# Research-Implementation/AudioVidSum-A-Multi-Modal-Approach-to-Video-Summarization

Hardware: AMD Instinct MI355X
Metric: frames/sec end-to-end (extract+fuse+score), 224x224 + 16kHz (higher is better)
Workload: dtype f16x2; 1 GPU; configs[1]: SumMe-shape batch, 25 videos x ~1800 frames (45143 frames/GPU), visual-only resnet50 extractor (batch-stat BN, the reference's 4-frame BatchNorm micro-batches inside each video) + AVBiLSTM attention scorer + mean-threshold selection; frames_per_gpu=45143, videos_per_gpu=25, extractor=resnet50, frames_per_group=4, chunk_frames=16384, parallelism=videos sharded x1, no data-path collective, selected_frames_rank0=22823

## Files before the change

### audiovidsum-a-multi-modal-approach-to-video-summarization_amd/csrc/igemm.hip

```cpp
#include "avs_internal.h"
#include "igemm_params.h"
#include <type_traits>

__device__ __attribute__((aligned(16))) unsigned int avs_zero16[4];

#ifdef AVS_STUDY
#define AVS_DEBUG_BIT(p, bit) ((p).debug & (bit))
#else
#define AVS_DEBUG_BIT(p, bit) 0
#endif

#define AVS_GLDS16(src, dst)                                                                        \
  __builtin_amdgcn_global_load_lds((const __attribute__((address_space(1))) void*)(src),            \
                                   (__attribute__((address_space(3))) void*)(dst), 16, 0, 0)

__device__ __forceinline__ void avs_split_bf16(const float4& p0, const float4& p1, bf16x8& hi, bf16x8& lo) {
  const float v[8] = {p0.x, p0.y, p0.z, p0.w, p1.x, p1.y, p1.z, p1.w};
  unsigned h[4], l[4];
#pragma unroll
  for (int j = 0; j < 4; ++j) {
    const unsigned short h0 = avs_f32_to_bf16(v[2 * j]), h1 = avs_f32_to_bf16(v[2 * j + 1]);
    const unsigned short l0 = avs_f32_to_bf16(v[2 * j] - avs_bf16_to_f32(h0));
    const unsigned short l1 = avs_f32_to_bf16(v[2 * j + 1] - avs_bf16_to_f32(h1));
    h[j] = (unsigned)h0 | ((unsigned)h1 << 16);
    l[j] = (unsigned)l0 | ((unsigned)l1 << 16);
  }
  hi = __builtin_bit_cast(bf16x8, make_uint4(h[0], h[1], h[2], h[3]));
  lo = __builtin_bit_cast(bf16x8, make_uint4(l[0], l[1], l[2], l[3]));
}


template <int ES, int BN, bool ACC64, bool SPATIAL, int ROWB, int EPI, bool PIPE, int WR = 2, bool FASTK = false,
          int SPLIT = 0, bool TAP9 = false, bool AP8 = false, bool XIN = false>
__global__ __launch_bounds__(256, (ROWB == 64 && !ACC64 && WR == 2) ? ((BN == 64 && ES == 2) ? 4 : 3) : 2) void igemm_kernel(
    IgemmParams p) {
  static_assert(!AP8 || (SPLIT == 2 && ES == 4 && PIPE && ROWB == 64 && FASTK && !SPATIAL && !TAP9 && EPI == EPI_STATS),
                "AVS_F16P8 input: the AVS_F16X2 1x1 convolution + statistics on the pipelined tiles");
  static_assert(!TAP9 || (((SPLIT == 2 && ES == 4) || (SPLIT == 0 && ES == 2)) && PIPE && WR == 4 && ROWB == 64 && FASTK &&
                          SPATIAL && (EPI == EPI_STATS || EPI == EPI_BNLOCAL || (EPI == EPI_BRELU && SPLIT == 2))),
                "the shifted-row form: AVS_F16X2 / bf16 convolution + statistics / tile-local BatchNorm (3x3), AVS_F16X2 bias + "
                "ReLU (any stride-1 'same' filter) on the pipelined 256-row tiles");
  static_assert(!XIN || (TAP9 && SPLIT == 2 && EPI == EPI_STATS), "the input affine: AVS_F16X2 nine-tap convolution + statistics");
  static_assert(SPLIT == 0 || (ES == 4 && !ACC64), "the split arithmetic is for 4-byte operands");
  static_assert(WR == 2 || (WR == 4 && !ACC64 && (ES == 2 || SPLIT != 0)),
                "256-row tiles are built for the bf16 variants and the fp32-split arithmetic");
  static_assert(!PIPE || (ROWB == 64 && !ACC64), "the 3-buffer pipeline is built for the 64-byte-row variants");
  static_assert(!ACC64 || (ES == 4 && BN == 64), "fp64 slice accumulation: fp32 operands, narrow tile only");
  static_assert(ROWB == 64 || ROWB == 128, "row bytes");
  constexpr int CE = 16 / ES;
  constexpr int BKE = ROWB / ES;
  constexpr int CPRR = ROWB / 16;
  constexpr int RPP = 256 / CPRR;
  constexpr int SH = ROWB == 128 ? 1 : 2;
  constexpr int KS = ROWB / 32;
  constexpr int WC = 4 / WR;
  constexpr int WCOLS = BN / WC;
  constexpr int A_ROWS = 64 * WR;
  constexpr int NA = A_ROWS / RPP;
  constexpr int NB = (BN + RPP - 1) / RPP;
  constexpr int NT = WCOLS / 32;
  constexpr int BUF = (A_ROWS + NB * RPP) * CPRR;
  static_assert(BN == 64 || BN == 128 || (BN == 96 && SPLIT == 2 && WR == 4 && PIPE && ROWB == 64 && EPI == EPI_BRELU),
                "96-column tiles: the AVS_F16X2 bias + ReLU form on the pipelined 256-row tiles");
  static_assert(WCOLS % 32 == 0, "a wave's columns are whole 32-wide MFMA tiles");
  constexpr int CT_PITCH = BN * 2 + 16;
  constexpr int CT_SLOTS = ES == 2 ? (A_ROWS * CT_PITCH) / 16 : 0;
  constexpr int NBUF = PIPE ? 3 : 2;
  constexpr int TAB_SLOTS = EPI == EPI_BNLOCAL ? (BNLOCAL_MAX_GROUPS * 2 * BN * 4) / 16
                            : EPI == EPI_STATS ? (WR * 2 * 2 * BN * 4) / 16
                                               : 0;
  constexpr int H2_P = WCOLS + 8;
  constexpr int H2_SLOTS = SPLIT == 2 ? (4 * 32 * H2_P * 4) / 16 : 0;
  constexpr int T9_AROWS = 384;
  constexpr int T9_ABUF = (T9_AROWS + 4) * CPRR;
  constexpr int T9_BBUF = NB * RPP * CPRR;
  constexpr int OPERAND_SLOTS = TAP9 ? 2 * T9_ABUF + 3 * T9_BBUF : NBUF * BUF;
  constexpr int LDS_BASE = OPERAND_SLOTS > CT_SLOTS + TAB_SLOTS ? OPERAND_SLOTS : CT_SLOTS + TAB_SLOTS;
  constexpr int LDS_SLOTS = LDS_BASE > H2_SLOTS ? LDS_BASE : H2_SLOTS;

  __shared__ uint4 lds[LDS_SLOTS];

  const unsigned nwg = gridDim.x, orig = blockIdx.x;
  const unsigned q = nwg >> 3, rr = nwg & 7, xcd = orig & 7;
  const unsigned wg = (xcd < rr ? xcd * (q + 1) : rr * (q + 1) + (xcd - rr) * q) + (orig >> 3);
  const int tn = wg % p.tiles_n;
  const int tm = wg / p.tiles_n;
  const int m0 = EPI == EPI_BNLOCAL ? tm * p.tile_rows : tm * A_ROWS;
  const int n0 = tn * BN;

  const long long z = blockIdx.z;
  const char* __restrict__ x = p.x + z * p.sA * ES;
  const char* __restrict__ w = p.w + z * p.sB * ES;
  char* __restrict__ y = p.y + z * p.sC * ES;
  const float* __restrict__ bias = p.bias ? p.bias + z * p.sBias : nullptr;
  const char* zsrc = reinterpret_cast<const char*>(avs_zero16);

  const int t = threadIdx.x;
  const int wave = __builtin_amdgcn_readfirstlane(t >> 6), lane = t & 63;
  const int c = t & (CPRR - 1);
  const int rb = t / CPRR;
  const int cq = c ^ ((rb >> SH) & (CPRR - 1));

  const char* a_base[NA];
  int hi0[NA], wi0[NA];
#pragma unroll
  for (int i = 0; i < NA; ++i) {
    int m = m0 + rb + RPP * i;
    if constexpr (EPI == EPI_BNLOCAL) {
      if (rb + RPP * i >= p.tile_rows) m = p.M;
    }
    if (m < p.M && p.lin_stride >= 0) {
      hi0[i] = 0;
      wi0[i] = 0;
      a_base[i] = x + (long long)m * p.lin_stride * ES;
    } else if (m < p.M) {
      const int n = m / p.HoWo;
      const int rem = m - n * p.HoWo;
      const int ho = rem / p.Wo;
      const int wo = rem - ho * p.Wo;
      hi0[i] = ho * p.sh - p.ph;
      wi0[i] = wo * p.sw - p.pw;
      a_base[i] = x + ((long long)n * p.x_img_stride + (long long)hi0[i] * p.x_row_stride +
                       (long long)wi0[i] * p.x_px_stride) * ES;
    } else {
      hi0[i] = -(1 << 29);
      wi0[i] = 0;
      a_base[i] = nullptr;
    }
  }
  const char* b_base[NB];
#pragma unroll
  for (int i = 0; i < NB; ++i) {
    const int n = n0 + rb + RPP * i;
// ... 110 lines not shown
#pragma unroll
    for (int i = 0; i < NA; ++i) {
      bool ok = kval && a_base[i] != nullptr;
      if constexpr (SPATIAL)
        ok = ok && (unsigned)(hi0[i] + kh) < (unsigned)p.H && (unsigned)(wi0[i] + kw) < (unsigned)p.W;
      const unsigned long long am = ok ? ~0ull : 0ull;
      const char* src = reinterpret_cast<const char*>(
          (reinterpret_cast<unsigned long long>(a_base[i] + koff) & am) |
          (reinterpret_cast<unsigned long long>(zsrc) & ~am));
      AVS_GLDS16(src, abuf + 256 * i);
    }
#pragma unroll
    for (int i = 0; i < NB; ++i) {
      const unsigned long long bm = (kval && b_base[i] != nullptr) ? ~0ull : 0ull;
      constexpr int KSE = 64 / ES;
      const char* bsrc = p.w_kstep ? w + (((long long)(kc / KSE) * p.N + (n0 + rb + RPP * i)) * KSE + (kc % KSE)) * ES
                                   : b_base[i] + (long long)kc * ES;
      const char* src = reinterpret_cast<const char*>((reinterpret_cast<unsigned long long>(bsrc) & bm) |
                                                      (reinterpret_cast<unsigned long long>(zsrc) & ~bm));
      AVS_GLDS16(src, bbuf + 256 * i);
    }
    kc += BKE;
    ci += BKE;
    while (ci >= p.cin) {
      ci -= p.cin;
      if (++kw == p.KW) {
        kw = 0;
        ++kh;
      }
    }
  };

  const int wr = wave / WC, wc = wave % WC;
  const int lr = lane & 31, lh = lane >> 5;

  f32x16 acc[2][NT];
#pragma unroll
  for (int i = 0; i < 2; ++i)
#pragma unroll
    for (int j = 0; j < NT; ++j)
#pragma unroll
      for (int e = 0; e < 16; ++e) acc[i][j][e] = 0.f;

  double acc64[ACC64 ? 2 : 1][ACC64 ? NT : 1][ACC64 ? 16 : 1];
  if constexpr (ACC64) {
#pragma unroll
    for (int i = 0; i < 2; ++i)
#pragma unroll
      for (int j = 0; j < NT; ++j)
#pragma unroll
        for (int e = 0; e < 16; ++e) acc64[i][j][e] = 0.0;
  }

  const int steps = (p.K + BKE - 1) / BKE;
  if constexpr (TAP9) {
    constexpr int T9_NA = T9_AROWS / RPP;
    constexpr bool TGEN = EPI == EPI_BRELU;
    const int ntap = TGEN ? p.K / p.cin : 9;
    const int tkw = TGEN ? p.KW : 3;
    const int tph = TGEN ? p.ph : 1, tpw = TGEN ? p.pw : 1;
    const long long pxs = TGEN ? p.x_px_stride : (long long)p.cin;
    const unsigned lds_base = (unsigned)(unsigned long long)((__attribute__((address_space(3))) char*)lds);
    const int w1 = TGEN ? tph * p.W + tpw : p.W + 1;
    const long long mbase = m0 > w1 ? m0 - w1 : 0;
    const __amdgpu_buffer_rsrc_t a9 = __builtin_amdgcn_make_buffer_rsrc(const_cast<char*>(x) + mbase * pxs * ES, 0,
                                                                         (int)BUF_OOB, 0x00020000);
    const __amdgpu_buffer_rsrc_t b9 = __builtin_amdgcn_make_buffer_rsrc(
        const_cast<char*>(w) + (p.w_kstep ? (long long)n0 * 64 : (long long)n0 * p.ldb * ES), 0, (int)BUF_OOB, 0x00020000);
    unsigned aoff9[T9_NA], boff9[NB];
#pragma unroll
    for (int i = 0; i < T9_NA; ++i) {
      const long long m = (long long)m0 - w1 + rb + RPP * i;
      aoff9[i] = (m >= 0 && m < p.M) ? (unsigned)((m - mbase) * pxs * ES) + cq * 16 : BUF_OOB;
    }
#pragma unroll
    for (int i = 0; i < NB; ++i)
      boff9[i] = (n0 + rb + RPP * i >= p.N || rb + RPP * i >= BN) ? BUF_OOB
                 : p.w_kstep                                      ? (unsigned)((rb + RPP * i) * 64) + (cq & 3) * 16
                                                                  : (unsigned)((long long)(rb + RPP * i) * p.ldb * ES) + cq * 16;
    unsigned vm[2];
#pragma unroll
    for (int mt = 0; mt < 2; ++mt) {
      unsigned mk = 0;
      const int m = m0 + wr * 64 + mt * 32 + lr;
      bool live = m < p.M;
      if constexpr (EPI == EPI_BNLOCAL) live = live && wr * 64 + mt * 32 + lr < p.tile_rows;
      if (live) {
        const int pix = m % p.HoWo;
        const int yy = pix / p.W, xx = pix - yy * p.W;
        if constexpr (TGEN) {
          for (int tp = 0; tp < ntap; ++tp)
            if ((unsigned)(yy + tp / tkw - tph) < (unsigned)p.H && (unsigned)(xx + tp % tkw - tpw) < (unsigned)p.W) mk |= 1u << tp;
        } else {
#pragma unroll
          for (int tp = 0; tp < 9; ++tp)
            if ((unsigned)(yy + tp / 3 - 1) < (unsigned)p.H && (unsigned)(xx + tp % 3 - 1) < (unsigned)p.W) mk |= 1u << tp;
        }
      }
      vm[mt] = mk;
    }
    if (t < 32) lds[(t >> 4) * T9_ABUF + T9_AROWS * CPRR + (t & 15)] = make_uint4(0u, 0u, 0u, 0u);
    asm volatile("s_waitcnt lgkmcnt(0)" ::: "memory");
    unsigned fb9[NT][2];
#pragma unroll
    for (int nt = 0; nt < NT; ++nt)
#pragma unroll
// ... 5 lines not shown
    const int nblk = p.cin / BKE;
    auto stage_a = [&](int blk, int buf) {
      uint4* abuf = lds + buf * T9_ABUF + wave * 64;
#pragma unroll
      for (int i = 0; i < T9_NA; ++i)
        __builtin_amdgcn_raw_ptr_buffer_load_lds(a9, (__attribute__((address_space(3))) void*)(abuf + 256 * i), 16,
                                                 (int)aoff9[i], blk * ROWB, 0, 0);
    };
    int sb_blk = 0, sb_tap = 0, sb_slot = 0;
    auto stage_b = [&]() {
      uint4* bbuf = lds + 2 * T9_ABUF + sb_slot * T9_BBUF + wave * 64;
      const int kstep = sb_tap * nblk + sb_blk;
      const int kb = p.w_kstep ? kstep * (p.N * ROWB) : kstep * ROWB;
#pragma unroll
      for (int i = 0; i < NB; ++i)
        __builtin_amdgcn_raw_ptr_buffer_load_lds(b9, (__attribute__((address_space(3))) void*)(bbuf + 256 * i), 16,
                                                 (int)boff9[i], kb, 0, 0);
      sb_slot = sb_slot == 2 ? 0 : sb_slot + 1;
      if (++sb_tap == ntap) {
        sb_tap = 0;
        ++sb_blk;
      }
    };
    auto xin_block = [&](int b) {
      uint4* ab = lds + (b & 1) * T9_ABUF;
#pragma unroll
      for (int i = 0; i < (T9_AROWS * 2) / 256; ++i) {
        const int u = t + 256 * i;
        const int a = u >> 1, run = u & 1;
        const int m = m0 - w1 + a;
        if (m < 0 || m >= p.M) continue;
        const int g = m / p.rows_per_group;
        const long long ch = (long long)g * p.cin + b * BKE + run * 8;
        uint4& hi = ab[a * CPRR + ((2 * run) ^ ((a >> SH) & (CPRR - 1)))];
        uint4& lo = ab[a * CPRR + ((2 * run + 1) ^ ((a >> SH) & (CPRR - 1)))];
        float v[8], sc[8], sf[8];
        avs_f16x2_join8(hi, lo, v);
        *reinterpret_cast<float4*>(&sc[0]) = *reinterpret_cast<const float4*>(p.in_scale + ch);
        *reinterpret_cast<float4*>(&sc[4]) = *reinterpret_cast<const float4*>(p.in_scale + ch + 4);
        *reinterpret_cast<float4*>(&sf[0]) = *reinterpret_cast<const float4*>(p.in_shift + ch);
        *reinterpret_cast<float4*>(&sf[4]) = *reinterpret_cast<const float4*>(p.in_shift + ch + 4);
#pragma unroll
        for (int j = 0; j < 8; ++j) v[j] = v[j] * sc[j] + sf[j];
        if (p.in_relu) {
#pragma unroll
          for (int j = 0; j < 8; ++j) v[j] = fmaxf(v[j], 0.f);
        }
        uint4 h, l;
        avs_f16x2_split8(v, h, l);
        hi = h;
        lo = l;
      }
    };
    stage_a(0, 0);
    stage_b();
    if (steps > 1) stage_b();
    const int abase = wr * 64 + lr + w1;
    int blk = 0, tap = 0, tdx = 0, slot = 0, sig = -w1;
    for (int s = 0; s < steps; ++s) {
      if (s + 1 < steps) {
        if (tap == 1 && blk + 1 < nblk)
          asm volatile("s_waitcnt vmcnt(%0)" ::"n"(NB + T9_NA) : "memory");
        else
          asm volatile("s_waitcnt vmcnt(%0)" ::"n"(NB) : "memory");
      } else {
        asm volatile("s_waitcnt vmcnt(0)" ::: "memory");
      }
      __builtin_amdgcn_s_barrier();
      if constexpr (XIN) {
        if (tap == 0) {
          xin_block(blk);
          asm volatile("s_waitcnt lgkmcnt(0)" ::: "memory");
          __builtin_amdgcn_s_barrier();
        }
      }
      const unsigned abuf = lds_base + (unsigned)(blk & 1) * (T9_ABUF * 16u);
      const unsigned bbase = lds_base + (unsigned)(2 * T9_ABUF + slot * T9_BBUF) * 16u;
      uint4 fa[2][2], fb[2][NT];
      unsigned aaddr[2];
#pragma unroll
      for (int mt = 0; mt < 2; ++mt) {
        const int a = ((vm[mt] >> tap) & 1u) ? abase + mt * 32 + sig : T9_AROWS;
        aaddr[mt] = abuf + (unsigned)a * ROWB + (unsigned)((SPLIT == 2 ? 2 * lh : lh) ^ ((a >> SH) & (CPRR - 1))) * 16u;
      }
#pragma unroll
      for (int mt = 0; mt < 2; ++mt) fa[0][mt] = avs_lds_read_b128(aaddr[mt]);
#pragma unroll
      for (int nt = 0; nt < NT; ++nt) fb[0][nt] = avs_lds_read_b128(bbase + fb9[nt][0]);
#pragma unroll
      for (int mt = 0; mt < 2; ++mt) fa[1][mt] = avs_lds_read_b128(aaddr[mt] ^ (SPLIT == 2 ? 16u : 32u));
#pragma unroll
      for (int nt = 0; nt < NT; ++nt) fb[1][nt] = avs_lds_read_b128(bbase + fb9[nt][1]);
      if (tap == 0 && blk + 1 < nblk) stage_a(blk + 1, (blk + 1) & 1);
      if (s + 2 < steps) stage_b();
      asm volatile("s_waitcnt lgkmcnt(%0)" ::"n"(2 + NT) : "memory");
#pragma unroll
      for (int mt = 0; mt < 2; ++mt) avs_pin(fa[0][mt]);
#pragma unroll
      for (int nt = 0; nt < NT; ++nt) avs_pin(fb[0][nt]);
      __builtin_amdgcn_sched_barrier(0);
#pragma unroll
      for (int mt = 0; mt < 2; ++mt)
#pragma unroll
        for (int nt = 0; nt < NT; ++nt)
          if constexpr (SPLIT == 2)
            acc[mt][nt] = __builtin_amdgcn_mfma_f32_32x32x16_f16(__builtin_bit_cast(avs_f16x8, fa[0][mt]),
                                                                 __builtin_bit_cast(avs_f16x8, fb[0][nt]), acc[mt][nt], 0, 0, 0);
          else
            acc[mt][nt] = __builtin_amdgcn_mfma_f32_32x32x16_bf16(__builtin_bit_cast(bf16x8, fa[0][mt]),
                                                                  __builtin_bit_cast(bf16x8, fb[0][nt]), acc[mt][nt], 0, 0, 0);
      asm volatile("s_waitcnt lgkmcnt(0)" ::: "memory");
#pragma unroll
      for (int mt = 0; mt < 2; ++mt) avs_pin(fa[1][mt]);
#pragma unroll
      for (int nt = 0; nt < NT; ++nt) avs_pin(fb[1][nt]);
      __builtin_amdgcn_sched_barrier(0);
#pragma unroll
      for (int mt = 0; mt < 2; ++mt)
#pragma unroll
        for (int nt = 0; nt < NT; ++nt) {
          if constexpr (SPLIT == 2) {
            acc[mt][nt] = __builtin_amdgcn_mfma_f32_32x32x16_f16(__builtin_bit_cast(avs_f16x8, fa[1][mt]),
                                                                 __builtin_bit_cast(avs_f16x8, fb[0][nt]), acc[mt][nt], 0, 0, 0);
            acc[mt][nt] = __builtin_amdgcn_mfma_f32_32x32x16_f16(__builtin_bit_cast(avs_f16x8, fa[0][mt]),
// ... 285 lines not shown
      } else {
#pragma unroll
        for (int mt = 0; mt < 2; ++mt)
#pragma unroll
          for (int e = 0; e < 16; ++e) {
            const int roff = mt * 32 + (e & 3) + 8 * (e >> 2);
            s += (roff >= lo && roff < hi) ? acc[mt][nt][e] : 0.f;
          }
      }
      return s + __shfl_xor(s, 32, 64);
    };
    auto wave_sq = [&](int nt, int lo, int hi, float mean) -> float {
      float s = 0.f;
#pragma unroll
      for (int mt = 0; mt < 2; ++mt)
#pragma unroll
        for (int e = 0; e < 16; ++e) {
          const int roff = mt * 32 + (e & 3) + 8 * (e >> 2);
          const float d = acc[mt][nt][e] - mean;
          s = (roff >= lo && roff < hi) ? fmaf(d, d, s) : s;
        }
      return s + __shfl_xor(s, 32, 64);
    };
    float sc0[NT], sf0[NT], sc1[NT], sf1[NT], sc2[NT], sf2[NT];
    int bnd1 = 1 << 30, bnd2 = 1 << 30;
    int used = A_ROWS;
    if constexpr (EPI == EPI_BNLOCAL) used = (m0 + p.tile_rows <= p.M ? p.tile_rows : p.M - m0);
    constexpr int G = WCOLS / 8;
    constexpr int RSTEP = 64 / G;
    constexpr int NU = (32 + RSTEP - 1) / RSTEP;
    constexpr bool RAGGED = 64 % G != 0;
    static_assert(!RAGGED || EPI == EPI_BRELU, "ragged run maps: the bias + ReLU form only (no residual rows)");
    constexpr bool NORM = EPI == EPI_BNLOCAL || EPI == EPI_AFFINE || EPI == EPI_BRELU;
    float* const wreg = fl + wave * (32 * H2_P);
    const bool relu = NORM && (EPI == EPI_BRELU || p.act == AVS_ACT_RELU);
    if constexpr (EPI == EPI_BRELU) {
#pragma unroll
      for (int nt = 0; nt < NT; ++nt) {
        const int col = n0 + wc * WCOLS + nt * 32 + lr;
        sc0[nt] = 1.f;
        sf0[nt] = col < p.N ? bias[col] : 0.f;
        sc1[nt] = sc2[nt] = 1.f;
        sf1[nt] = sf2[nt] = 0.f;
      }
    }
    const int rl0 = lane / G, grp = lane % G;
    const int col8 = n0 + wc * WCOLS + grp * 8;
    const int row_lim = (EPI == EPI_BNLOCAL ? m0 + used : p.M);
    const bool col_ok = col8 < p.N && (!RAGGED || lane < RSTEP * G);
    const bool relu_l = relu && (p.relu_cols <= 0 || col8 < p.relu_cols);
    const int p8_hi = (col8 >> 4) * 48 + ((col8 >> 3) & 1) * 16;
    const int p8_rem = 32 - ((col8 >> 3) & 1) * 8;
    uint4 rhi[2][NORM ? NU : 1], rlo[2][NORM ? NU : 1];
    auto res_fetch = [&](auto half) {
      constexpr int mt = decltype(half)::value;
      if constexpr (NORM) {
        const long long row0 = (long long)m0 + wr * 64 + mt * 32 + rl0;
        if (EPI == EPI_AFFINE && p.res_p8) {
          const char* base = p.residual + row0 * p.ldr * 3 + p8_hi;
          const long long step = (long long)RSTEP * p.ldr * 3;
#pragma unroll
          for (int it = 0; it < NU; ++it) {
            const bool ok = col_ok && row0 + it * RSTEP < row_lim;
            const char* rp = ok ? base + it * step : p.residual + p8_hi;
            rhi[mt][it] = *reinterpret_cast<const uint4*>(rp);
            const uint2 q = *reinterpret_cast<const uint2*>(rp + p8_rem);
            rlo[mt][it] = make_uint4(q.x, q.y, 0u, 0u);
          }
          return;
        }
        const char* base = p.residual + (row0 * p.ldr + col8) * 4;
        const long long step = (long long)RSTEP * p.ldr * 4;
#pragma unroll
        for (int it = 0; it < NU; ++it) {
          const bool ok = col_ok && row0 + it * RSTEP < row_lim;
          const uint4* rp = reinterpret_cast<const uint4*>(ok ? base + it * step : p.residual);
          rhi[mt][it] = rp[0];
          rlo[mt][it] = rp[1];
        }
      }
    };
    if (NORM && p.residual) res_fetch(std::integral_constant<int, 0>{});
    if constexpr (EPI == EPI_STATS) {
      const int rpg = p.rows_per_group;
      float* const T1 = fl;
      float* const T2 = fl + WR * 2 * BN;
      const int tile_end = (m0 + A_ROWS < p.M ? m0 + A_ROWS : p.M);
      const int r_first = m0 + wr * 64;
      const bool live = r_first < p.M;
      int g0 = 0, g1 = -1, r_end = r_first;
      if (live) {
        r_end = (r_first + 64 < p.M ? r_first + 64 : p.M);
        g0 = r_first / rpg;
        g1 = (r_end - 1) / rpg;
      }
      for (int g = g0; g <= g1; ++g) {
        const int lo = (g * rpg > r_first ? g * rpg : r_first) - r_first - 4 * lh;
        const int hi = ((g + 1) * rpg < r_end ? (g + 1) * rpg : r_end) - r_first - 4 * lh;
#pragma unroll
        for (int nt = 0; nt < NT; ++nt) {
          const float s = wave_sum(nt, lo, hi);
          if (lh == 0) T1[(wr * 2 + (g - g0)) * BN + wc * WCOLS + nt * 32 + lr] = s;
        }
      }
      __syncthreads();
      auto tile_total = [&](const float* T, int g, int cc) -> float {
        float s = 0.f;
#pragma unroll
        for (int r = 0; r < WR; ++r) {
          const int rf = m0 + r * 64;
          if (rf >= p.M) break;
          const int re = (rf + 64 < p.M ? rf + 64 : p.M);
          const int a = rf / rpg, b = (re - 1) / rpg;
          if (g >= a && g <= b) s += T[(r * 2 + (g - a)) * BN + cc];
        }
        return s;
      };
      for (int g = g0; g <= g1; ++g) {
        const int lo = (g * rpg > r_first ? g * rpg : r_first) - r_first - 4 * lh;
        const int hi = ((g + 1) * rpg < r_end ? (g + 1) * rpg : r_end) - r_first - 4 * lh;
        const int n_g = ((g + 1) * rpg < tile_end ? (g + 1) * rpg : tile_end) - (g * rpg > m0 ? g * rpg : m0);
#pragma unroll
        for (int nt = 0; nt < NT; ++nt) {
          const int cc = wc * WCOLS + nt * 32 + lr;
          const float mean = tile_total(T1, g, cc) / (float)n_g;
          const float s = wave_sq(nt, lo, hi, mean);
          if (lh == 0) T2[(wr * 2 + (g - g0)) * BN + cc] = s;
        }
      }
      __syncthreads();
      {
        const int g_lo = m0 / rpg;
        const int nj = (tile_end - 1) / rpg - g_lo + 1;
        for (int i = t; i < nj * BN; i += 256) {
          const int j = i / BN, cc = i - j * BN;
// ... 35 lines not shown
#pragma unroll
        for (int r = 0; r < WR; ++r) {
          if (r * 64 >= used) break;
          const int re = (r * 64 + 64 < used ? r * 64 + 64 : used);
          const int a = (r * 64) / rpg, b = (re - 1) / rpg;
          if (k >= a && k <= b) s += R[(r * ng + k) * BN + cc];
        }
        return s;
      };
      const float inv_n = 1.f / (float)rpg;
      for (int k = k0; k <= k1; ++k) {
        const int lo = (k * rpg > w_first ? k * rpg : w_first) - w_first - 4 * lh;
        const int hi = ((k + 1) * rpg < w_end ? (k + 1) * rpg : w_end) - w_first - 4 * lh;
#pragma unroll
        for (int nt = 0; nt < NT; ++nt) {
          const int cc = wc * WCOLS + nt * 32 + lr;
          const float s = wave_sq(nt, lo, hi, tile_total(R1, k, cc) * inv_n);
          if (lh == 0) R2[(wr * ng + k) * BN + cc] = s;
        }
      }
      __syncthreads();
      for (int i = t; i < ng * BN; i += 256) {
        const int k = i / BN, cc = i - k * BN;
        const float mean = tile_total(R1, k, cc) * inv_n;
        const float var = tile_total(R2, k, cc) * inv_n;
        const int col = n0 + cc;
        const float sc = (col < p.N ? p.gamma[col] : 0.f) / sqrtf(var + p.eps);
        TAB[(2 * k) * BN + cc] = sc;
        TAB[(2 * k + 1) * BN + cc] = (col < p.N ? p.beta[col] : 0.f) - mean * sc;
      }
      __syncthreads();
      {
        const int kmax = ng > 0 ? ng - 1 : 0;
        const int kb0 = k0 < kmax ? k0 : kmax;
        const int kb1 = kb0 + 1 < kmax ? kb0 + 1 : kmax, kb2 = kb0 + 2 < kmax ? kb0 + 2 : kmax;
        bnd1 = (kb0 + 1) * rpg - w_first - 4 * lh;
        bnd2 = bnd1 + rpg;
#pragma unroll
        for (int nt = 0; nt < NT; ++nt) {
          const int cc = wc * WCOLS + nt * 32 + lr;
          sc0[nt] = TAB[(2 * kb0) * BN + cc], sf0[nt] = TAB[(2 * kb0 + 1) * BN + cc];
          sc1[nt] = TAB[(2 * kb1) * BN + cc], sf1[nt] = TAB[(2 * kb1 + 1) * BN + cc];
          sc2[nt] = TAB[(2 * kb2) * BN + cc], sf2[nt] = TAB[(2 * kb2 + 1) * BN + cc];
        }
      }
      __syncthreads();
    }
    if constexpr (EPI == EPI_AFFINE) {
      const int rpg = p.rows_per_group;
      const int r_first = m0 + wr * 64;
      const int gl = (p.M - 1) / rpg;
      const int ga = r_first / rpg < gl ? r_first / rpg : gl;
      const int gb = ga + 1 < gl ? ga + 1 : gl, gc = ga + 2 < gl ? ga + 2 : gl;
      bnd1 = (ga + 1) * rpg - r_first - 4 * lh;
      bnd2 = bnd1 + rpg;
#pragma unroll
      for (int nt = 0; nt < NT; ++nt) {
        const int col = n0 + wc * WCOLS + nt * 32 + lr;
        const bool cv = col < p.N;
        sc0[nt] = cv ? p.gamma[(long long)ga * p.N + col] : 0.f, sf0[nt] = cv ? p.beta[(long long)ga * p.N + col] : 0.f;
        sc1[nt] = cv ? p.gamma[(long long)gb * p.N + col] : 0.f, sf1[nt] = cv ? p.beta[(long long)gb * p.N + col] : 0.f;
        sc2[nt] = cv ? p.gamma[(long long)gc * p.N + col] : 0.f, sf2[nt] = cv ? p.beta[(long long)gc * p.N + col] : 0.f;
      }
    }
    if constexpr (NORM) {
#pragma unroll
      for (int mt = 0; mt < 2; ++mt)
#pragma unroll
        for (int nt = 0; nt < NT; ++nt)
#pragma unroll
          for (int e = 0; e < 16; ++e) {
            const int roff = mt * 32 + (e & 3) + 8 * (e >> 2);
            const bool in1 = roff >= bnd1, in2 = roff >= bnd2;
            const float sc = in2 ? sc2[nt] : (in1 ? sc1[nt] : sc0[nt]);
            const float sf = in2 ? sf2[nt] : (in1 ? sf1[nt] : sf0[nt]);
            acc[mt][nt][e] = fmaf(acc[mt][nt][e], sc, sf);
          }
    }
#pragma unroll
    for (int mt = 0; mt < 2; ++mt) {
#pragma unroll
      for (int nt = 0; nt < NT; ++nt)
#pragma unroll
        for (int e = 0; e < 16; ++e)
          wreg[((e & 3) + 8 * (e >> 2) + 4 * lh) * H2_P + nt * 32 + lr] = acc[mt][nt][e];
      if (mt == 0 && NORM && p.residual) res_fetch(std::integral_constant<int, 1>{});
      asm volatile("s_waitcnt lgkmcnt(0)" ::: "memory");
      __builtin_amdgcn_wave_barrier();
      const long long row0 = (long long)m0 + wr * 64 + mt * 32 + rl0;
      char* ybase = y + (row0 * p.ldc + col8) * 4;
      long long ystep = (long long)RSTEP * p.ldc * 4;
      if (p.nsplit > 0 && col8 >= p.nsplit) {
        ybase = p.y2 + (row0 * p.ldc2 + (col8 - p.nsplit)) * 4;
        ystep = (long long)RSTEP * p.ldc2 * 4;
      }
#pragma unroll
      for (int it = 0; it < NU; ++it) {
        const float* src = wreg + (rl0 + it * RSTEP) * H2_P + grp * 8;
        const float4 f0 = *reinterpret_cast<const float4*>(src);
        const float4 f1 = *reinterpret_cast<const float4*>(src + 4);
        const long long row = row0 + it * RSTEP;
        if (!(col_ok && row < row_lim)) continue;
        if constexpr (RAGGED) {
          if (rl0 + it * RSTEP >= 32) continue;
        }
        float v[8] = {f0.x, f0.y, f0.z, f0.w, f1.x, f1.y, f1.z, f1.w};
        if constexpr (NORM) {
          if (p.residual) {
            float rv[8];
            avs_pin(rhi[mt][it]);
            avs_pin(rlo[mt][it]);
            if (EPI == EPI_AFFINE && p.res_p8)
              avs_f16p8_join8(rhi[mt][it], make_uint2(rlo[mt][it].x, rlo[mt][it].y), rv);
            else
              avs_f16x2_join8(rhi[mt][it], rlo[mt][it], rv);
            if constexpr (EPI == EPI_AFFINE) {
              if (p.res_scale) {
                const long long gq = (row / p.rows_per_group) * p.N + col8;
                const float4 a0 = *reinterpret_cast<const float4*>(p.res_scale + gq);
                const float4 a1 = *reinterpret_cast<const float4*>(p.res_scale + gq + 4);
                const float4 b0 = *reinterpret_cast<const float4*>(p.res_shift + gq);
                const float4 b1 = *reinterpret_cast<const float4*>(p.res_shift + gq + 4);
                const float as[8] = {a0.x, a0.y, a0.z, a0.w, a1.x, a1.y, a1.z, a1.w};
                const float bs[8] = {b0.x, b0.y, b0.z, b0.w, b1.x, b1.y, b1.z, b1.w};
#pragma unroll
                for (int j = 0; j < 8; ++j) rv[j] = fmaf(rv[j], as[j], bs[j]);
              }
            }
#pragma unroll
            for (int j = 0; j < 8; ++j) v[j] += rv[j];
          }
          if (relu_l) {
#pragma unroll
            for (int j = 0; j < 8; ++j) v[j] = fmaxf(v[j], 0.f);
          }
        }
        if (EPI == EPI_AFFINE && p.y_p8) {
          uint4 hi;
          uint2 rem;
          avs_f16p8_split8(v, hi, rem);
          char* dst = y + (row * p.ldc) * 3 + p8_hi;
          *reinterpret_cast<uint4*>(dst) = hi;
          *reinterpret_cast<uint2*>(dst + p8_rem) = rem;
          continue;
        }
        uint4 hi, lo;
        avs_f16x2_split8(v, hi, lo);
        uint4* dst = reinterpret_cast<uint4*>(ybase + it * ystep);
        dst[0] = hi;
        dst[1] = lo;
      }
      asm volatile("s_waitcnt lgkmcnt(0)" ::: "memory");
      __builtin_amdgcn_wave_barrier();
    }
  } else {
  constexpr int E_CPRW = BN / 8;
  constexpr int E_RSTEP = 256 / E_CPRW;
  constexpr int E_NIT = A_ROWS / E_RSTEP;
  float* const sred = reinterpret_cast<float*>(reinterpret_cast<char*>(lds) + (size_t)CT_SLOTS * 16);
  if constexpr (EPI == EPI_STATS) {
    const int r_first = m0 + wr * 64;
    if (r_first < p.M) {
      const int r_last = (r_first + 63 < p.M ? r_first + 63 : p.M - 1);
      const int g0 = r_first / p.rows_per_group, g1 = r_last / p.rows_per_group;
#pragma unroll
      for (int nt = 0; nt < NT; ++nt) {
        const int cc = wc * WCOLS + nt * 32 + lr;
        if (g0 == g1) {
          float s1 = 0.f, s2 = 0.f;
#pragma unroll
          for (int mt = 0; mt < 2; ++mt)
#pragma unroll
            for (int e = 0; e < 16; ++e) {
              const float v = acc[mt][nt][e];
              s1 += v;
              s2 = fmaf(v, v, s2);
            }
          s1 += __shfl_xor(s1, 32, 64);
          s2 += __shfl_xor(s2, 32, 64);
// ... 604 lines not shown
                        : igemm_lift_form<ES, BN, ACC64, SP, ROWB, PIPE, 4, false>(pl, grid, stream, p);
    }
    if constexpr (BN != 96) {
      if (pl.wr == 2)
        return pl.fastk ? igemm_lift_form<ES, BN, ACC64, SP, ROWB, PIPE, 2, true>(pl, grid, stream, p)
                        : igemm_lift_form<ES, BN, ACC64, SP, ROWB, PIPE, 2, false>(pl, grid, stream, p);
    }
    return false;
  }
}

template <int ES, int BN, bool ACC64, bool SP, int ROWB>
static bool igemm_lift_pipe(const IgemmPlan& pl, dim3 grid, hipStream_t stream, const IgemmParams& p) {
  if constexpr (ROWB == 64 && !ACC64) {
    if (pl.pipe) return igemm_lift_tile<ES, BN, ACC64, SP, ROWB, true>(pl, grid, stream, p);
  }
  if constexpr (BN != 96) {
    if (!pl.pipe) return igemm_lift_tile<ES, BN, ACC64, SP, ROWB, false>(pl, grid, stream, p);
  }
  return false;
}

template <int ES, int BN, bool ACC64>
static bool igemm_lift(const IgemmPlan& pl, dim3 grid, hipStream_t stream, const IgemmParams& p) {
  if (pl.es != ES || pl.bn != BN || pl.acc64 != ACC64) return false;
  if (pl.rowb == 64)
    return pl.spatial ? igemm_lift_pipe<ES, BN, ACC64, true, 64>(pl, grid, stream, p)
                      : igemm_lift_pipe<ES, BN, ACC64, false, 64>(pl, grid, stream, p);
  if constexpr (BN != 96) {
    if (pl.rowb == 128)
      return pl.spatial ? igemm_lift_pipe<ES, BN, ACC64, true, 128>(pl, grid, stream, p)
                        : igemm_lift_pipe<ES, BN, ACC64, false, 128>(pl, grid, stream, p);
  }
  return false;
}

static int igemm_run(const IgemmPlan& pl, IgemmParams& p, hipStream_t stream, const char* who) {
  if (pl.operand_checks >= 1 && pl.dtype == AVS_F16X2)
    AVS_REQUIRE(((((uintptr_t)p.x) | ((uintptr_t)p.w) | ((uintptr_t)p.y)) & 31u) == 0, AVS_E_ALIGN,
                "%s: AVS_F16X2 operands must be 32-byte aligned", who);
  if (pl.operand_checks >= 2) {
    AVS_REQUIRE(p.x && p.w && p.y, AVS_E_ARG, "%s: null operand", who);
    AVS_REQUIRE(p.bias_mode == AVS_BIAS_NONE || p.bias, AVS_E_ARG, "%s: bias mode %d without bias", who, p.bias_mode);
  }
  if (pl.operand_checks >= 3)
    AVS_REQUIRE(avs_aligned16(p.x) && avs_aligned16(p.w), AVS_E_ALIGN, "%s: x / w must be 16-byte aligned", who);
  if (pl.status != AVS_OK) return pl.status;
  if (pl.grid == 0) return AVS_OK;
  p.split = pl.split;
  p.tall = pl.tall;
  p.tiles_n = pl.tiles_n;
  p.lin_stride = pl.lin_stride;
#ifdef AVS_STUDY
  p.debug = g_debug_flags;
#endif
  const dim3 grid((unsigned)pl.grid, 1, (unsigned)pl.batch);
  if (pl.local224) {
    igemm_h2_local224_launch(p, pl.spatial, grid, stream);
    AVS_CHECK_LAUNCH(who);
    return AVS_OK;
  }
  const bool launched = igemm_lift<2, 64, false>(pl, grid, stream, p) || igemm_lift<2, 128, false>(pl, grid, stream, p) ||
                        igemm_lift<4, 64, true>(pl, grid, stream, p) || igemm_lift<4, 64, false>(pl, grid, stream, p) ||
                        igemm_lift<4, 96, false>(pl, grid, stream, p) || igemm_lift<4, 128, false>(pl, grid, stream, p);
  AVS_REQUIRE(launched, AVS_E_UNSUPPORTED,
              "%s: no kernel for this plan (dtype %d, %d x %d tile, K = %d, N = %d, variant %d, %d-byte steps, epilogue %d, pipe %d, "
              "fastk %d, tap9 %d, ap8 %d, xin %d): nothing was launched", who, pl.dtype, pl.wr * 64, pl.bn, p.K, p.N, p.variant,
              pl.rowb, pl.epi, pl.pipe, pl.fastk, pl.tap9, pl.ap8, pl.in_affine);
  AVS_CHECK_LAUNCH(who);
  return AVS_OK;
}

static int igemm_launch(int dtype, IgemmParams& p, int batch, hipStream_t stream, const char* who) {
  IgemmPlan pl;
  igemm_plan(dtype, p, batch, p.stat_part != nullptr, p.in_scale != nullptr, who, pl);
  return igemm_run(pl, p, stream, who);
}

static int conv_geometry(const avs_conv_desc* d, bool has_bias, IgemmParams& p, const char* who) {
  AVS_REQUIRE(d != nullptr, AVS_E_ARG, "%s: null descriptor", who);
  AVS_REQUIRE(d->n >= 0 && d->h > 0 && d->w > 0 && d->cin > 0 && d->kh > 0 && d->kw > 0 && d->sh > 0 && d->sw > 0 &&
                  d->ph >= 0 && d->pw >= 0 && d->ho > 0 && d->wo > 0 && d->cout > 0,
              AVS_E_SHAPE, "%s: non-positive extent", who);
  AVS_REQUIRE((d->ho - 1) * d->sh - d->ph + d->kh - 1 < d->h + d->ph &&
                  (d->wo - 1) * d->sw - d->pw + d->kw - 1 < d->w + d->pw,
              AVS_E_SHAPE, "%s: output extent %dx%d exceeds what input %dx%d allows", who, d->ho, d->wo, d->h, d->w);
  const long long rows = (long long)d->n * d->ho * d->wo;
  AVS_REQUIRE(rows < (1ll << 31), AVS_E_SHAPE, "%s: %lld output pixels exceed int32", who, rows);
  p.M = (int)rows;
  p.N = d->cout;
  p.K = d->kh * d->kw * d->cin;
  p.HoWo = d->ho * d->wo;
  p.Wo = d->wo;
  p.H = d->h;
  p.W = d->w;
  p.cin = d->cin;
  p.KW = d->kw;
  p.sh = d->sh;
  p.sw = d->sw;
  p.ph = d->ph;
  p.pw = d->pw;
  p.x_img_stride = d->x_img_stride;
  p.x_row_stride = d->x_row_stride;
  p.x_px_stride = d->x_px_stride;
  p.ldb = d->w_row_stride;
  AVS_REQUIRE(d->w_layout == AVS_W_ROWS || d->w_layout == AVS_W_KSTEP32, AVS_E_ARG, "%s: bad w_layout %d", who,
              d->w_layout);
// ... 388 lines not shown
```

### audiovidsum-a-multi-modal-approach-to-video-summarization_amd/csrc/igemm_params.h

```cpp
#pragma once
#include "avs_internal.h"

typedef __bf16 bf16x8 __attribute__((ext_vector_type(8)));
typedef float f32x16 __attribute__((ext_vector_type(16)));

struct IgemmParams {
  const char* x;
  const char* w;
  char* y;
  const float* bias;
  int M, N, K;
  int HoWo, Wo, H, W, cin, KW;
  int sh, sw, ph, pw;
  long long x_img_stride, x_row_stride, x_px_stride;
  long long ldb, ldc;
  long long sA, sB, sC, sBias;
  float alpha;
  int act, bias_mode;
  int tiles_n;
  float* stat_part;
  int stat_slots;
  int rows_per_group;
  long long lin_stride;
  const float* gamma;
// ... 4 lines not shown
  int split;
  int tall;
  int w_kstep;
  int tile_rows;
  int affine;
  const float* res_scale;
  const float* res_shift;
  int variant;
  int x_p8, y_p8, res_p8;
  char* y2;
  long long ldc2;
  int nsplit;
  int relu_cols;
  int cluster;
  unsigned epoch;
  unsigned long long* xchg;
  unsigned* xerr;
  int packed;
  const float* in_scale;
  const float* in_shift;
  int in_relu;
#ifdef AVS_STUDY
  int debug;
#endif
};

enum { EPI_PLAIN = 0, EPI_STATS = 1, EPI_ANY = 2, EPI_BRELU = 3, EPI_BNLOCAL = 5, EPI_AFFINE = 6 };
constexpr int BNLOCAL_MAX_GROUPS = 6;
constexpr int STATS_MIN_GROUP_ROWS = 64;

typedef unsigned u32x4 __attribute__((ext_vector_type(4)));
typedef unsigned u32x2 __attribute__((ext_vector_type(2)));
__device__ __forceinline__ void avs_pin(uint4& v) {
  u32x4 r = __builtin_bit_cast(u32x4, v);
  asm volatile("" : "+v"(r));
  v = __builtin_bit_cast(uint4, r);
}

__device__ __forceinline__ void avs_pin2(uint2& v) {
  u32x2 r = __builtin_bit_cast(u32x2, v);
  asm volatile("" : "+v"(r));
  v = __builtin_bit_cast(uint2, r);
}
__device__ __forceinline__ uint2 avs_lds_read_b64(unsigned byte_addr) {
  uint2 v;
  asm volatile("ds_read_b64 %0, %1" : "=v"(v) : "v"(byte_addr));
  return v;
}
__device__ __forceinline__ uint4 avs_lds_read_b128(unsigned byte_addr) {
  uint4 v;
  asm volatile("ds_read_b128 %0, %1" : "=v"(v) : "v"(byte_addr));
  return v;
}

struct IgemmPlan {
  int status;
  int operand_checks;
  int dtype, batch;
  int es;
  int split;
  int bn;
  bool acc64;
  bool tall;
  bool spatial;
  long long lin_stride;
  int rowb;
  int epi;
  bool pipe;
  int wr;
  bool fastk;
  bool tap9, ap8, xin;
  bool in_affine;
  bool local224;
  int tile_rows;
  long long tiles_m;
  int tiles_n;
  long long grid;
};

inline bool igemm_buffer_window_ok(const IgemmParams& p, long long lin_stride, int es, int bn) {
  const long long rows = 256;
  long long extent;
  if (lin_stride >= 0)
    extent = rows * lin_stride + p.K;
  else
    extent = (rows / p.HoWo + 2) * p.x_img_stride + (long long)(p.K / (p.cin * p.KW) + p.ph) * p.x_row_stride +
             (long long)(p.KW + p.pw) * p.x_px_stride + p.cin;
  return extent * es < (1ll << 31) && (long long)bn * p.ldb * es + (long long)p.K * es < (1ll << 31) &&
         p.x_img_stride >= 0 && p.x_row_stride >= 0 && p.x_px_stride >= 0;
}

bool igemm_h2_local224_ok(const IgemmParams& p, int dtype, long long lin_stride);
void igemm_h2_local224_launch(const IgemmParams& p, bool spatial, dim3 grid, hipStream_t stream);
```

Baseline: 27590 frames/s.

## Hoist epilogue affine/residual loads before main loop and stage res_scale/in-affine tables in LDS

Adds an early-load path to the split-2 pipelined affine-epilogue GEMM. It fetches per-group gamma/beta, and optionally the first residual rows, before the K loop, so their global latency overlaps the MMA work instead of stalling the epilogue. When a wave's 64 rows fall in one BN group, res_scale/res_shift are loaded once and kept in LDS rather than re-read from global per row. A study-only path stages the input-affine scale/shift in an LDS table, which adds LDS and register pressure. Without study flags, the early path runs only when no residual is present, while the LDS res_scale table is used whenever a residual and res_scale are present and the rows fit in one group.

Measured after the change: 27620 frames/s (median of 6 runs). About the same (+0.1%).

```diff
diff --git a/audiovidsum-a-multi-modal-approach-to-video-summarization_amd/csrc/igemm.hip b/audiovidsum-a-multi-modal-approach-to-video-summarization_amd/csrc/igemm.hip
--- a/audiovidsum-a-multi-modal-approach-to-video-summarization_amd/csrc/igemm.hip
+++ b/audiovidsum-a-multi-modal-approach-to-video-summarization_amd/csrc/igemm.hip
@@ -6,8 +6,10 @@
 
 #ifdef AVS_STUDY
 #define AVS_DEBUG_BIT(p, bit) ((p).debug & (bit))
+constexpr bool AVS_STUDY_BUILD = true;
 #else
 #define AVS_DEBUG_BIT(p, bit) 0
+constexpr bool AVS_STUDY_BUILD = false;
 #endif
 
 #define AVS_GLDS16(src, dst)                                                                        \
@@ -78,7 +80,12 @@
   constexpr int LDS_BASE = OPERAND_SLOTS > CT_SLOTS + TAB_SLOTS ? OPERAND_SLOTS : CT_SLOTS + TAB_SLOTS;
   constexpr int LDS_SLOTS = LDS_BASE > H2_SLOTS ? LDS_BASE : H2_SLOTS;
 
-  __shared__ uint4 lds[LDS_SLOTS];
+  constexpr bool XT = XIN && AVS_STUDY_BUILD;
+  constexpr int XT_CIN = 128;
+  constexpr int XT_SLOTS = XT ? (2 * 2 * XT_CIN * 4) / 16 : 0;
+  static_assert(!XIN || (LDS_SLOTS + XT_SLOTS) * 16 <= 80 * 1024, "the input-affine form: two workgroups per CU");
+
+  __shared__ uint4 lds[LDS_SLOTS + XT_SLOTS];
 
   const unsigned nwg = gridDim.x, orig = blockIdx.x;
   const unsigned q = nwg >> 3, rr = nwg & 7, xcd = orig & 7;
@@ -295,6 +302,53 @@
         for (int e = 0; e < 16; ++e) acc64[i][j][e] = 0.0;
   }
 
+  constexpr bool EARLY = SPLIT == 2 && EPI == EPI_AFFINE && PIPE;
+  constexpr int EA_G = WCOLS / 8, EA_RSTEP = 64 / EA_G, EA_NU = (32 + EA_RSTEP - 1) / EA_RSTEP;
+  constexpr int EA_NE = !EARLY ? 0 : (EA_NU <= 4 ? EA_NU : EA_NU / 2);
+  float ea_aff[EARLY ? 6 : 1][NT];
+  uint4 ea_rhi[EA_NE > 0 ? EA_NE : 1], ea_rlo[EA_NE > 0 ? EA_NE : 1];
+  int ea_bnd1 = 1 << 30;
+  bool early = false;
+  if constexpr (EARLY) {
+    early = (!p.residual || AVS_DEBUG_BIT(p, 2048)) && !AVS_DEBUG_BIT(p, 256);
+    if (early) {
+      const int rpg = p.rows_per_group;
+      const int r_first = m0 + wr * 64;
+      const int gl = (p.M - 1) / rpg;
+      const int ga = r_first / rpg < gl ? r_first / rpg : gl;
+      const int gb = ga + 1 < gl ? ga + 1 : gl, gc = ga + 2 < gl ? ga + 2 : gl;
+      ea_bnd1 = (ga + 1) * rpg - r_first - 4 * lh;
+#pragma unroll
+      for (int nt = 0; nt < NT; ++nt) {
+        const int col = n0 + wc * WCOLS + nt * 32 + lr;
+        const bool cv = col < p.N;
+        ea_aff[0][nt] = cv ? p.gamma[(long long)ga * p.N + col] : 0.f, ea_aff[1][nt] = cv ? p.beta[(long long)ga * p.N + col] : 0.f;
+        ea_aff[2][nt] = cv ? p.gamma[(long long)gb * p.N + col] : 0.f, ea_aff[3][nt] = cv ? p.beta[(long long)gb * p.N + col] : 0.f;
+        ea_aff[4][nt] = cv ? p.gamma[(long long)gc * p.N + col] : 0.f, ea_aff[5][nt] = cv ? p.beta[(long long)gc * p.N + col] : 0.f;
+      }
+      if (p.residual) {
+        const int rl0 = lane / EA_G, col8 = n0 + wc * WCOLS + (lane % EA_G) * 8;
+        const long long row0 = (long long)m0 + wr * 64 + rl0;
+        const bool col_ok = col8 < p.N;
+        const int p8_hi = (col8 >> 4) * 48 + ((col8 >> 3) & 1) * 16, p8_rem = 32 - ((col8 >> 3) & 1) * 8;
+#pragma unroll
+        for (int it = 0; it < EA_NE; ++it) {
+          const bool ok = col_ok && row0 + it * EA_RSTEP < p.M;
+          if (p.res_p8) {
+            const char* rp = ok ? p.residual + (row0 + it * EA_RSTEP) * p.ldr * 3 + p8_hi : p.residual + p8_hi;
+            ea_rhi[it] = *reinterpret_cast<const uint4*>(rp);
+            const uint2 q = *reinterpret_cast<const uint2*>(rp + p8_rem);
+            ea_rlo[it] = make_uint4(q.x, q.y, 0u, 0u);
+          } else {
+            const uint4* rp = reinterpret_cast<const uint4*>(ok ? p.residual + ((row0 + it * EA_RSTEP) * p.ldr + col8) * 4 : p.residual);
+            ea_rhi[it] = rp[0];
+            ea_rlo[it] = rp[1];
+          }
+        }
+      }
+    }
+  }
+
   const int steps = (p.K + BKE - 1) / BKE;
   if constexpr (TAP9) {
     constexpr int T9_NA = T9_AROWS / RPP;
@@ -406,9 +460,84 @@
         lo = l;
       }
     };
+    bool xt_on = false;
+    unsigned xt_row[XT ? 3 : 1], xt_aff[XT ? 3 : 1];
+    bool xt_ok[XT ? 3 : 1];
+    float4 xt_src = make_float4(0.f, 0.f, 0.f, 0.f);
+    const unsigned xt_base = lds_base + (unsigned)LDS_SLOTS * 16u;
+    if constexpr (XT) {
+      const long long mf = (long long)m0 - w1 > 0 ? (long long)m0 - w1 : 0;
+      const long long ml = (long long)m0 - w1 + T9_AROWS - 1 < p.M - 1 ? (long long)m0 - w1 + T9_AROWS - 1 : p.M - 1;
+      const int gf = (int)mf / p.rows_per_group, gn = (int)ml / p.rows_per_group;
+      xt_on = gn - gf <= 1 && p.cin <= XT_CIN && !AVS_DEBUG_BIT(p, 1024);
+      if (xt_on) {
+#pragma unroll
+        for (int i = 0; i < 3; ++i) {
+          const int a = (t + 256 * i) >> 1, run = t & 1;
+          const long long m = (long long)m0 - w1 + a;
+          xt_ok[i] = m >= 0 && m < p.M;
+          const int sel = xt_ok[i] ? (int)m / p.rows_per_group - gf : 0;
+          xt_row[i] = (unsigned)(a * CPRR + ((2 * run) ^ ((a >> SH) & (CPRR - 1)))) * 16u;
+          xt_aff[i] = (unsigned)(sel * 2 * p.cin + run * 8) * 4u;
+        }
+        if (t < p.cin) {
+          const int e = 4 * t, sel = e / (2 * p.cin), k = (e / p.cin) & 1, ch = e % p.cin;
+          const int g = gf + sel < gn ? gf + sel : gn;
+          xt_src = *reinterpret_cast<const float4*>((k ? p.in_shift : p.in_scale) + (long long)g * p.cin + ch);
+        }
+      }
+    }
+    auto xin_block_tab = [&](int b) {
+      const unsigned ab = lds_base + (unsigned)(b & 1) * (T9_ABUF * 16u);
+      const unsigned tb = xt_base + (unsigned)(b * BKE) * 4u;
+      uint4 dh[3], dl[3], qs[3][2], qf[3][2];
+#pragma unroll
+      for (int i = 0; i < 3; ++i) {
+        dh[i] = avs_lds_read_b128(ab + xt_row[i]);
+        dl[i] = avs_lds_read_b128(ab + (xt_row[i] ^ 16u));
+      }
+#pragma unroll
+      for (int i = 0; i < 3; ++i) {
+        qs[i][0] = avs_lds_read_b128(tb + xt_aff[i]);
+        qs[i][1] = avs_lds_read_b128(tb + xt_aff[i] + 16u);
+        qf[i][0] = avs_lds_read_b128(tb + xt_aff[i] + (unsigned)p.cin * 4u);
+        qf[i][1] = avs_lds_read_b128(tb + xt_aff[i] + (unsigned)p.cin * 4u + 16u);
+      }
+      asm volatile("s_waitcnt lgkmcnt(0)" ::: "memory");
+#pragma unroll
+      for (int i = 0; i < 3; ++i) {
+        avs_pin(dh[i]), avs_pin(dl[i]), avs_pin(qs[i][0]), avs_pin(qs[i][1]), avs_pin(qf[i][0]), avs_pin(qf[i][1]);
+      }
+#pragma unroll
+      for (int i = 0; i < 3; ++i) {
+        if (!xt_ok[i]) continue;
+        float v[8];
+        avs_f16x2_join8(dh[i], dl[i], v);
+        const float4 s0 = __builtin_bit_cast(float4, qs[i][0]), s1 = __builtin_bit_cast(float4, qs[i][1]);
+        const float4 f0 = __builtin_bit_cast(float4, qf[i][0]), f1 = __builtin_bit_cast(float4, qf[i][1]);
+        const float sc[8] = {s0.x, s0.y, s0.z, s0.w, s1.x, s1.y, s1.z, s1.w};
+        const float sf[8] = {f0.x, f0.y, f0.z, f0.w, f1.x, f1.y, f1.z, f1.w};
+#pragma unroll
+        for (int j = 0; j < 8; ++j) v[j] = v[j] * sc[j] + sf[j];
+        if (p.in_relu) {
+#pragma unroll
+          for (int j = 0; j < 8; ++j) v[j] = fmaxf(v[j], 0.f);
+        }
+        uint4 h, l;
+        avs_f16x2_split8(v, h, l);
+        avs_lds_write_b128(ab + xt_row[i], h);
+        avs_lds_write_b128(ab + (xt_row[i] ^ 16u), l);
+      }
+    };
     stage_a(0, 0);
     stage_b();
     if (steps > 1) stage_b();
+    if constexpr (XT) {
+      if (xt_on) {
+        if (t < p.cin) avs_lds_write_b128(xt_base + 16u * t, __builtin_bit_cast(uint4, xt_src));
+        asm volatile("s_waitcnt lgkmcnt(0)" ::: "memory");
+      }
+    }
     const int abase = wr * 64 + lr + w1;
     int blk = 0, tap = 0, tdx = 0, slot = 0, sig = -w1;
     for (int s = 0; s < steps; ++s) {
@@ -423,7 +552,10 @@
       __builtin_amdgcn_s_barrier();
       if constexpr (XIN) {
         if (tap == 0) {
-          xin_block(blk);
+          if (XT && xt_on)
+            xin_block_tab(blk);
+          else
+            xin_block(blk);
           asm volatile("s_waitcnt lgkmcnt(0)" ::: "memory");
           __builtin_amdgcn_s_barrier();
         }
@@ -815,15 +947,16 @@
     const int p8_hi = (col8 >> 4) * 48 + ((col8 >> 3) & 1) * 16;
     const int p8_rem = 32 - ((col8 >> 3) & 1) * 8;
     uint4 rhi[2][NORM ? NU : 1], rlo[2][NORM ? NU : 1];
-    auto res_fetch = [&](auto half) {
+    auto res_fetch = [&](auto half, auto from) {
       constexpr int mt = decltype(half)::value;
+      constexpr int IT0 = decltype(from)::value;
       if constexpr (NORM) {
         const long long row0 = (long long)m0 + wr * 64 + mt * 32 + rl0;
         if (EPI == EPI_AFFINE && p.res_p8) {
           const char* base = p.residual + row0 * p.ldr * 3 + p8_hi;
           const long long step = (long long)RSTEP * p.ldr * 3;
 #pragma unroll
-          for (int it = 0; it < NU; ++it) {
+          for (int it = IT0; it < NU; ++it) {
             const bool ok = col_ok && row0 + it * RSTEP < row_lim;
             const char* rp = ok ? base + it * step : p.residual + p8_hi;
             rhi[mt][it] = *reinterpret_cast<const uint4*>(rp);
@@ -835,7 +968,7 @@
         const char* base = p.residual + (row0 * p.ldr + col8) * 4;
         const long long step = (long long)RSTEP * p.ldr * 4;
 #pragma unroll
-        for (int it = 0; it < NU; ++it) {
+        for (int it = IT0; it < NU; ++it) {
           const bool ok = col_ok && row0 + it * RSTEP < row_lim;
           const uint4* rp = reinterpret_cast<const uint4*>(ok ? base + it * step : p.residual);
           rhi[mt][it] = rp[0];
@@ -843,7 +976,37 @@
         }
       }
     };
-    if (NORM && p.residual) res_fetch(std::integral_constant<int, 0>{});
+    constexpr bool RS_TAB = EPI == EPI_AFFINE && !(WR == 4 && BN == 128);
+    static_assert(!RS_TAB || 4 * 32 * H2_P + 4 * G * 16 <= LDS_SLOTS * 4, "the res_scale | res_shift runs fit behind the staging regions");
+    float* const rtab = fl + 4 * 32 * H2_P + wave * (G * 16) + grp * 16;
+    float rs_q[RS_TAB ? 16 : 1];
+    bool rs_one = false;
+    if constexpr (RS_TAB) {
+      if (p.residual && p.res_scale && !AVS_DEBUG_BIT(p, 512)) {
+        const int rpg = p.rows_per_group, gl = (p.M - 1) / rpg;
+        const int rbase = m0 + wr * 64;
+        const int gq = rbase / rpg;
+        const long long rend = (long long)rbase + 64 < p.M ? (long long)rbase + 64 : p.M;
+        rs_one = rend <= (long long)(gq + 1) * rpg;
+        const long long q0 = (long long)(gq < gl ? gq : gl) * p.N + (col_ok ? col8 : 0);
+        const float4 a0 = *reinterpret_cast<const float4*>(p.res_scale + q0);
+        const float4 a1 = *reinterpret_cast<const float4*>(p.res_scale + q0 + 4);
+        const float4 b0 = *reinterpret_cast<const float4*>(p.res_shift + q0);
+        const float4 b1 = *reinterpret_cast<const float4*>(p.res_shift + q0 + 4);
+        const float q[16] = {a0.x, a0.y, a0.z, a0.w, a1.x, a1.y, a1.z, a1.w, b0.x, b0.y, b0.z, b0.w, b1.x, b1.y, b1.z, b1.w};
+#pragma unroll
+        for (int j = 0; j < 16; ++j) rs_q[j] = q[j];
+      }
+    }
+    if (NORM && p.residual) {
+      if (EARLY && early) {
+#pragma unroll
+        for (int it = 0; it < EA_NE; ++it) rhi[0][it] = ea_rhi[it], rlo[0][it] = ea_rlo[it];
+        res_fetch(std::integral_constant<int, 0>{}, std::integral_constant<int, EA_NE>{});
+      } else {
+        res_fetch(std::integral_constant<int, 0>{}, std::integral_constant<int, 0>{});
+      }
+    }
     if constexpr (EPI == EPI_STATS) {
       const int rpg = p.rows_per_group;
       float* const T1 = fl;
@@ -985,15 +1148,26 @@
       const int gl = (p.M - 1) / rpg;
       const int ga = r_first / rpg < gl ? r_first / rpg : gl;
       const int gb = ga + 1 < gl ? ga + 1 : gl, gc = ga + 2 < gl ? ga + 2 : gl;
-      bnd1 = (ga + 1) * rpg - r_first - 4 * lh;
-      bnd2 = bnd1 + rpg;
-#pragma unroll
-      for (int nt = 0; nt < NT; ++nt) {
-        const int col = n0 + wc * WCOLS + nt * 32 + lr;
-        const bool cv = col < p.N;
-        sc0[nt] = cv ? p.gamma[(long long)ga * p.N + col] : 0.f, sf0[nt] = cv ? p.beta[(long long)ga * p.N + col] : 0.f;
-        sc1[nt] = cv ? p.gamma[(long long)gb * p.N + col] : 0.f, sf1[nt] = cv ? p.beta[(long long)gb * p.N + col] : 0.f;
-        sc2[nt] = cv ? p.gamma[(long long)gc * p.N + col] : 0.f, sf2[nt] = cv ? p.beta[(long long)gc * p.N + col] : 0.f;
+      if (EARLY && early) {
+        bnd1 = ea_bnd1;
+        bnd2 = bnd1 + rpg;
+#pragma unroll
+        for (int nt = 0; nt < NT; ++nt) {
+          sc0[nt] = ea_aff[0][nt], sf0[nt] = ea_aff[1][nt];
+          sc1[nt] = ea_aff[2][nt], sf1[nt] = ea_aff[3][nt];
+          sc2[nt] = ea_aff[4][nt], sf2[nt] = ea_aff[5][nt];
+        }
+      } else {
+        bnd1 = (ga + 1) * rpg - r_first - 4 * lh;
+        bnd2 = bnd1 + rpg;
+#pragma unroll
+        for (int nt = 0; nt < NT; ++nt) {
+          const int col = n0 + wc * WCOLS + nt * 32 + lr;
+          const bool cv = col < p.N;
+          sc0[nt] = cv ? p.gamma[(long long)ga * p.N + col] : 0.f, sf0[nt] = cv ? p.beta[(long long)ga * p.N + col] : 0.f;
+          sc1[nt] = cv ? p.gamma[(long long)gb * p.N + col] : 0.f, sf1[nt] = cv ? p.beta[(long long)gb * p.N + col] : 0.f;
+          sc2[nt] = cv ? p.gamma[(long long)gc * p.N + col] : 0.f, sf2[nt] = cv ? p.beta[(long long)gc * p.N + col] : 0.f;
+        }
       }
     }
     if constexpr (NORM) {
@@ -1017,7 +1191,14 @@
 #pragma unroll
         for (int e = 0; e < 16; ++e)
           wreg[((e & 3) + 8 * (e >> 2) + 4 * lh) * H2_P + nt * 32 + lr] = acc[mt][nt][e];
-      if (mt == 0 && NORM && p.residual) res_fetch(std::integral_constant<int, 1>{});
+      if (mt == 0 && NORM && p.residual) res_fetch(std::integral_constant<int, 1>{}, std::integral_constant<int, 0>{});
+      if constexpr (RS_TAB) {
+        if (mt == 0 && rs_one && rl0 == 0) {
+#pragma unroll
+          for (int k = 0; k < 4; ++k)
+            *reinterpret_cast<float4*>(rtab + 4 * k) = make_float4(rs_q[4 * k], rs_q[4 * k + 1], rs_q[4 * k + 2], rs_q[4 * k + 3]);
+        }
+      }
       asm volatile("s_waitcnt lgkmcnt(0)" ::: "memory");
       __builtin_amdgcn_wave_barrier();
       const long long row0 = (long long)m0 + wr * 64 + mt * 32 + rl0;
@@ -1049,15 +1230,24 @@
               avs_f16x2_join8(rhi[mt][it], rlo[mt][it], rv);
             if constexpr (EPI == EPI_AFFINE) {
               if (p.res_scale) {
-                const long long gq = (row / p.rows_per_group) * p.N + col8;
-                const float4 a0 = *reinterpret_cast<const float4*>(p.res_scale + gq);
-                const float4 a1 = *reinterpret_cast<const float4*>(p.res_scale + gq + 4);
-                const float4 b0 = *reinterpret_cast<const float4*>(p.res_shift + gq);
-                const float4 b1 = *reinterpret_cast<const float4*>(p.res_shift + gq + 4);
-                const float as[8] = {a0.x, a0.y, a0.z, a0.w, a1.x, a1.y, a1.z, a1.w};
-                const float bs[8] = {b0.x, b0.y, b0.z, b0.w, b1.x, b1.y, b1.z, b1.w};
-#pragma unroll
-                for (int j = 0; j < 8; ++j) rv[j] = fmaf(rv[j], as[j], bs[j]);
+                if (rs_one) {
+                  const float4 a0 = *reinterpret_cast<const float4*>(rtab), a1 = *reinterpret_cast<const float4*>(rtab + 4);
+                  const float4 b0 = *reinterpret_cast<const float4*>(rtab + 8), b1 = *reinterpret_cast<const float4*>(rtab + 12);
+                  const float as[8] = {a0.x, a0.y, a0.z, a0.w, a1.x, a1.y, a1.z, a1.w};
+                  const float bs[8] = {b0.x, b0.y, b0.z, b0.w, b1.x, b1.y, b1.z, b1.w};
+#pragma unroll
+                  for (int j = 0; j < 8; ++j) rv[j] = fmaf(rv[j], as[j], bs[j]);
+                } else {
+                  const long long gq = (row / p.rows_per_group) * p.N + col8;
+                  const float4 a0 = *reinterpret_cast<const float4*>(p.res_scale + gq);
+                  const float4 a1 = *reinterpret_cast<const float4*>(p.res_scale + gq + 4);
+                  const float4 b0 = *reinterpret_cast<const float4*>(p.res_shift + gq);
+                  const float4 b1 = *reinterpret_cast<const float4*>(p.res_shift + gq + 4);
+                  const float as[8] = {a0.x, a0.y, a0.z, a0.w, a1.x, a1.y, a1.z, a1.w};
+                  const float bs[8] = {b0.x, b0.y, b0.z, b0.w, b1.x, b1.y, b1.z, b1.w};
+#pragma unroll
+                  for (int j = 0; j < 8; ++j) rv[j] = fmaf(rv[j], as[j], bs[j]);
+                }
               }
             }
 #pragma unroll
@@ -1768,7 +1958,8 @@
   p.tiles_n = pl.tiles_n;
   p.lin_stride = pl.lin_stride;
 #ifdef AVS_STUDY
-  p.debug = g_debug_flags;
+  const int early_off = getenv("AVS_EARLY_LOADS_OFF") ? atoi(getenv("AVS_EARLY_LOADS_OFF")) & 15 : 4;
+  p.debug = g_debug_flags | (early_off << 8);
 #endif
   const dim3 grid((unsigned)pl.grid, 1, (unsigned)pl.batch);
   if (pl.local224) {
diff --git a/audiovidsum-a-multi-modal-approach-to-video-summarization_amd/csrc/igemm_params.h b/audiovidsum-a-multi-modal-approach-to-video-summarization_amd/csrc/igemm_params.h
--- a/audiovidsum-a-multi-modal-approach-to-video-summarization_amd/csrc/igemm_params.h
+++ b/audiovidsum-a-multi-modal-approach-to-video-summarization_amd/csrc/igemm_params.h
@@ -80,6 +80,10 @@
   asm volatile("ds_read_b128 %0, %1" : "=v"(v) : "v"(byte_addr));
   return v;
 }
+__device__ __forceinline__ void avs_lds_write_b128(unsigned byte_addr, const uint4& v) {
+  const u32x4 r = __builtin_bit_cast(u32x4, v);
+  asm volatile("ds_write_b128 %0, %1" ::"v"(byte_addr), "v"(r) : "memory");
+}
 
 struct IgemmPlan {
   int status;
```
